# LiXirong/pytorch-r2d2

Measured on AMD Instinct MI355X. Metric: learner_steps_per_sec, higher is better.
Workload: dtype fp32; 1 GPU; model=r2d2-qnet (reference model.py: conv32x3 + LSTM256 + dueling, 6 actions), preset=atari57, global_batch=64, per_gpu_batch=64, seq_len=80, burn_in=40, n_step=5, target_mode=fixed, matmul=bf16x3 split (fp32 accumulate, fp32 state/storage), replay_rows_per_gpu=999936, parallelism=dp1, hip_graph=True, hoisted_step=True, graph_chunk=8

## Files before the change

### csrc/kernels/optim.hip

```cpp
#include "../common.h"
#include "../pack_step.h"
#include "../rms_pack.h"
#include "../adam_elem.h"

__global__ void rmsprop_centered_kernel(float* __restrict__ p, const float* __restrict__ g,
                                        float* __restrict__ sq, float* __restrict__ ga, int64_t n,
                                        float lr, float alpha, float eps, float gscale,
                                        const float* __restrict__ clip_sumsq, float max_norm) {
  float scale = gscale;
  if (clip_sumsq != nullptr && max_norm > 0.f) {
    const float norm = sqrtf(*clip_sumsq) * gscale;
    if (norm > max_norm) scale *= max_norm / (norm + 1e-6f);
  }
  const int64_t n4 = n >> 2;
  const int64_t stride = (int64_t)gridDim.x * blockDim.x;
  for (int64_t i = blockIdx.x * (int64_t)blockDim.x + threadIdx.x; i < n4; i += stride) {
    f32x4 pv = ((f32x4*)p)[i], gv = ((const f32x4*)g)[i];
    f32x4 sv = ((f32x4*)sq)[i], av = ((f32x4*)ga)[i];
#pragma unroll
    for (int e = 0; e < 4; ++e) {
      float s = sv[e], m = av[e];
      pv[e] = rms_elem(s, m, pv[e], gv[e] * scale, lr, alpha, eps);
      sv[e] = s;
      av[e] = m;
    }
    ((f32x4*)p)[i] = pv;
    ((f32x4*)sq)[i] = sv;
    ((f32x4*)ga)[i] = av;
  }
  for (int64_t i = (n4 << 2) + blockIdx.x * (int64_t)blockDim.x + threadIdx.x; i < n; i += stride) {
    float sv = sq[i], av = ga[i];
    p[i] = rms_elem(sv, av, p[i], g[i] * scale, lr, alpha, eps);
    sq[i] = sv;
    ga[i] = av;
  }
}

__global__ __launch_bounds__(256) void rmsprop_pack_kernel(const RmsPackArgs a) {
  const int b = (int)blockIdx.x - a.tblocks;
  if (b < 0) {
    rmsprop_torso_items(a, blockIdx.x);
    return;
  }
  rmsprop_pack_items(a, b * (int64_t)blockDim.x + threadIdx.x, (int64_t)(gridDim.x - a.tblocks) * blockDim.x);
}

__global__ void adam_kernel(float* __restrict__ p, const float* __restrict__ g,
                            float* __restrict__ m, float* __restrict__ v, int64_t n, float lr,
                            float b1, float b2, float eps, float gscale,
                            const int64_t* __restrict__ step, const float* __restrict__ clip_sumsq,
                            float max_norm) {
  float scale = gscale;
  if (clip_sumsq != nullptr && max_norm > 0.f) {
    const float norm = sqrtf(*clip_sumsq) * gscale;
    if (norm > max_norm) scale *= max_norm / (norm + 1e-6f);
  }
  const AdamCoef c = adam_coef(lr, b1, b2, eps, step, 1);
  const int64_t stride = (int64_t)gridDim.x * blockDim.x;
  for (int64_t i = blockIdx.x * (int64_t)blockDim.x + threadIdx.x; i < n; i += stride) {
    float mi = m[i], vi = v[i];
    const float pn = adam_elem(mi, vi, p[i], g[i] * scale, c);
    m[i] = mi;
    v[i] = vi;
    p[i] = pn;
  }
}

__global__ __launch_bounds__(256) void adam_pack_kernel(const RmsPackArgs a, float b2, int step_off) {
  const AdamUpd u{adam_coef(a.lr, a.alpha, b2, a.eps, a.step, step_off)};
  const int b = (int)blockIdx.x - a.tblocks;
  if (b < 0) {
    opt_torso_items(a, blockIdx.x, u);
    return;
  }
  opt_pack_items(a, b * (int64_t)blockDim.x + threadIdx.x, (int64_t)(gridDim.x - a.tblocks) * blockDim.x, u);
}

__global__ void sumsq_kernel(const float* __restrict__ g, int64_t n, float* __restrict__ out) {
  float s = 0.f;
  const int64_t stride = (int64_t)gridDim.x * blockDim.x;
  for (int64_t i = blockIdx.x * (int64_t)blockDim.x + threadIdx.x; i < n; i += stride) s += g[i] * g[i];
  s = wave_sum(s);
  if ((threadIdx.x & 63) == 0) atomicAdd(out, s);
}

constexpr int GSQ_MAX_FLAT = 256;
static inline int gsq_flat_blocks(int64_t quads) {
  int64_t b = (quads + 255) / 256;
  return (int)(b > GSQ_MAX_FLAT ? GSQ_MAX_FLAT : b);
}

__device__ __forceinline__ float gsq_block_sum(float s, float* red) {
  s = wave_sum(s);
  __syncthreads();
  if ((threadIdx.x & 63) == 0) red[threadIdx.x >> 6] = s;
  __syncthreads();
  return ((red[0] + red[1]) + red[2]) + red[3];
}

__global__ __launch_bounds__(256) void grad_sumsq_kernel(
    const float* __restrict__ g, int64_t quads, float* __restrict__ out, float* partials,
    unsigned* ticket, const float* __restrict__ slab, int G, int SL, const int* __restrict__ dst,
    const float* __restrict__ scale, float* __restrict__ gw, int tblocks) {
  __shared__ float part[4][64];
  __shared__ float red[4];
  __shared__ int last;
  float s = 0.f;
  const int b = (int)blockIdx.x - tblocks;
// ... 159 lines not shown
extern "C" int r2_adam_pack(float* p, const float* g, float* m, float* v, int64_t n, float lr,
                            float b1, float b2, float eps, float gscale, const float* clip_sumsq,
                            float max_norm, const int* dst4, bf16* bf, bf16* bf_t, int64_t lo_off,
                            float* target, const int64_t* step, int64_t interval, int step_off,
                            void* stream) {
  RmsPackArgs a{p, g, m, v, n, lr, b1, eps, gscale, clip_sumsq, max_norm, dst4, bf, bf_t,
                lo_off, target, step, interval};
  if (!rms_pack_args_ok(a)) return -1;
  hipLaunchKernelGGL(adam_pack_kernel, dim3(grid_for(n, 4)), dim3(256), 0, (hipStream_t)stream, a,
                     b2, step_off);
  R2_CHECK_LAUNCH();
  return 0;
}

extern "C" int r2_adam_pack_slab(float* p, float* g, float* m, float* v, int64_t n, float lr,
                                 float b1, float b2, float eps, float gscale, const int* dst4,
                                 bf16* bf, bf16* bf_t, int64_t lo_off, float* target,
                                 const int64_t* step, int64_t interval, int step_off,
                                 const float* slab, int grid, int SL, const int* dst,
                                 const float* scale, int64_t tq, void* stream) {
  RmsPackArgs a{p, g, m, v, n, lr, b1, eps, gscale, nullptr, 0.f, dst4, bf, bf_t,
                lo_off, target, step, interval};
  a.slab = slab; a.tdst = dst; a.tscale = scale; a.gw = g;
  a.tG = grid; a.tSL = SL; a.tblocks = (SL + 63) / 64; a.tq = tq;
  if (!rms_pack_args_ok(a) || !slab || !dst || !scale || grid <= 0 || SL <= 0 || tq < 0 ||
      4 * tq > n)
    return -1;
  hipLaunchKernelGGL(adam_pack_kernel, dim3(a.tblocks + grid_for(4 * tq, 4)), dim3(256), 0,
                     (hipStream_t)stream, a, b2, step_off);
  R2_CHECK_LAUNCH();
  return 0;
}

extern "C" int r2_pack_bf16(const float* src, const int* idx, bf16* out, int64_t n, void* stream) {
  hipLaunchKernelGGL(pack_bf16_kernel, dim3(grid_for(n, 2)), dim3(256), 0, (hipStream_t)stream, src,
                     idx, out, n);
  R2_CHECK_LAUNCH();
  return 0;
}

extern "C" int r2_pack_split(const float* src, const int* idx, bf16* out, int64_t n,
                             int64_t lo_off, void* stream) {
  hipLaunchKernelGGL(pack_split_kernel, dim3(grid_for(n, 2)), dim3(256), 0, (hipStream_t)stream,
                     src, idx, out, n, lo_off);
  R2_CHECK_LAUNCH();
  return 0;
}

extern "C" int r2_gather_f32(const float* src, const int* idx, float* out, int64_t n, void* stream) {
  hipLaunchKernelGGL(gather_f32_kernel, dim3(grid_for(n, 2)), dim3(256), 0, (hipStream_t)stream,
                     src, idx, out, n);
  R2_CHECK_LAUNCH();
  return 0;
}

extern "C" int r2_copy_if_due(float* dst, const float* src, int64_t n, const int64_t* step,
                              int64_t interval, void* stream) {
  hipLaunchKernelGGL(copy_if_due_kernel, dim3(grid_for(n, 4)), dim3(256), 0, (hipStream_t)stream,
                     dst, src, n, step, interval);
  R2_CHECK_LAUNCH();
  return 0;
}

__global__ void pack_step_kernel(const PackStepArgs a) {
  pack_step_items(a, blockIdx.x * (int64_t)blockDim.x + threadIdx.x, (int64_t)gridDim.x * blockDim.x);
}
// ... 16 lines not shown
```

### csrc/rms_pack.h

```cpp
#pragma once
#include "common.h"
#include "slab_reduce.h"

struct RmsPackArgs {
  float* p;
  const float* g;
  float* sq;
  float* ga;
  int64_t n;
  float lr, alpha, eps, gscale;
  const float* clip_sumsq;
  float max_norm;
  const int* dst4;
  bf16* bf;
  bf16* bf_t;
  int64_t lo_off;
  float* target;
  const int64_t* step;
  int64_t interval;
  const float* slab;
  const int* tdst;
  const float* tscale;
  float* gw;
  int tG, tSL, tblocks, pad_;
  int64_t tq;
};

__device__ __forceinline__ float rms_elem(float& sq, float& ga, float p, float gr, float lr,
                                          float alpha, float eps) {
  sq = alpha * sq + (1.f - alpha) * gr * gr;
  ga = alpha * ga + (1.f - alpha) * gr;
  return p - lr * gr / (sqrtf(sq - ga * ga) + eps);
}

struct RmsUpd {
  float lr, alpha, eps;
  __device__ __forceinline__ float operator()(float& sq, float& ga, float p, float gr) const {
    return rms_elem(sq, ga, p, gr, lr, alpha, eps);
  }
};

template <class Upd>
__device__ __forceinline__ void opt_pack_items(const RmsPackArgs& a, int64_t first, int64_t stride,
                                               const Upd upd) {
  float scale = a.gscale;
  if (a.clip_sumsq != nullptr && a.max_norm > 0.f) {
    const float norm = sqrtf(*a.clip_sumsq) * a.gscale;
    if (norm > a.max_norm) scale *= a.max_norm / (norm + 1e-6f);
  }
  float* __restrict__ p = a.p;
  const float* __restrict__ g = a.g;
  float* __restrict__ sq = a.sq;
  float* __restrict__ ga = a.ga;
  const bool due = a.interval <= 1 || ((*a.step) + 1) % a.interval == 0;
  const int64_t n = a.n, n4 = n >> 2;
  auto quad = [&](int64_t q) {
    f32x4 pv = ((f32x4*)p)[q], gv = ((const f32x4*)g)[q];
    f32x4 sv = ((f32x4*)sq)[q], av = ((f32x4*)ga)[q];
    const int d = a.dst4[q];
#pragma unroll
    for (int e = 0; e < 4; ++e) {
      float s = sv[e], m = av[e];
      pv[e] = upd(s, m, pv[e], gv[e] * scale);
      sv[e] = s;
      av[e] = m;
    }
    ((f32x4*)p)[q] = pv;
    ((f32x4*)sq)[q] = sv;
    ((f32x4*)ga)[q] = av;
    if (due) ((f32x4*)a.target)[q] = pv;
    if (d >= 0) {
      bf16x4 h, l;
#pragma unroll
      for (int e = 0; e < 4; ++e) {
        h[e] = (bf16)pv[e];
        l[e] = (bf16)(pv[e] - (float)h[e]);
      }
      *(bf16x4*)(a.bf + d) = h;
      if (a.lo_off) *(bf16x4*)(a.bf + a.lo_off + d) = l;
      if (due) {
        *(bf16x4*)(a.bf_t + d) = h;
        if (a.lo_off) *(bf16x4*)(a.bf_t + a.lo_off + d) = l;
      }
    }
  };
  const int64_t qend = a.tblocks ? a.tq : n4;
  for (int64_t i = first; i < qend; i += stride) quad(i);
  for (int64_t i = (n4 << 2) + first; i < n && !a.tblocks; i += stride) {
    float sv = sq[i], av = ga[i];
    p[i] = upd(sv, av, p[i], g[i] * scale);
    sq[i] = sv;
    ga[i] = av;
    if (due) a.target[i] = p[i];
  }
}

__device__ __forceinline__ void rmsprop_pack_items(const RmsPackArgs& a, int64_t first, int64_t stride) {
  opt_pack_items(a, first, stride, RmsUpd{a.lr, a.alpha, a.eps});
}

template <class Upd>
__device__ __forceinline__ void opt_torso_items(const RmsPackArgs& a, int blk, const Upd upd) {
  __shared__ float part[4][64];
  const float s = slab_column_sum(a.slab, a.tG, a.tSL, blk, part);
  const int e = blk * 64 + (int)threadIdx.x;
  if (threadIdx.x >= 64 || e >= a.tSL) return;
  const int m = a.tdst[e];
  const float gv = s * a.tscale[e];
  a.gw[m] = gv;
  float sv = a.sq[m], av = a.ga[m];
  const float pv = upd(sv, av, a.p[m], gv * a.gscale);
  a.sq[m] = sv;
  a.ga[m] = av;
  a.p[m] = pv;
  if (a.interval <= 1 || ((*a.step) + 1) % a.interval == 0) a.target[m] = pv;
}

__device__ __forceinline__ void rmsprop_torso_items(const RmsPackArgs& a, int blk) {
  opt_torso_items(a, blk, RmsUpd{a.lr, a.alpha, a.eps});
}

inline bool rms_pack_args_ok(const RmsPackArgs& a) {
  return !((((uintptr_t)a.p | (uintptr_t)a.g | (uintptr_t)a.sq | (uintptr_t)a.ga | (uintptr_t)a.target) & 15) ||
           (((uintptr_t)a.bf | (uintptr_t)a.bf_t) & 7) || (a.lo_off & 3) || !a.dst4 || !a.step);
}
```

### pytorch_r2d2_amd/config.py

```python
from __future__ import annotations

import copy
import dataclasses
from dataclasses import dataclass, field
from typing import Any, Dict, Optional


@dataclass
class EnvConfig:
    name: str = "synthetic"
    action_repeat: int = 4
    n_stacks: int = 4
    frame_h: int = 84
    frame_w: int = 84
    channels_per_frame: int = 1
    n_actions: int = 6
    episode_len: int = 400
    switch: int = 8
    cue_only_first: bool = False
    obs_dim: int = 4
    pong_points: int = 21
    pong_max_steps: int = 5000
    pong_opp_lapse: int = 64
    breakout_lives: int = 5
# ... 43 lines not shown
    adam_betas: tuple = (0.9, 0.999)
    grad_clip: float = 0.0
    value_rescale: bool = False
    value_rescale_eps: float = 1e-3
    target_update_interval: int = 1000
    publish_interval: int = 100
    ingest_interval: int = 20
    checkpoint_interval: int = 10_000
    initial_exploration: int = 50_000
    target_mode: str = "shifted"
    compute_dtype: str = "bf16"
    lstm_impl: str = "persistent"
    lstm_handoff: str = "tagged"
    bwd_gemm: str = "group"
    fuse_opt_pack: bool = True
    fold_torso_reduce: bool = True
    td_fuse_head_bwd: bool = True
    td_fuse_head_fwd: bool = True
    td_fuse_dh: bool = True
    lstm_xcd_pairs: bool = True
    sp_gemm: str = "fused"
    sp_group_splits: str = "auto"
    sp_group_cfg: int = -2
    sp_head_grads_in_bptt: bool = True
    torso_bwd: str = "fused"
    conv_autotune: bool = True
    use_graph: bool = True
    bptt_dh: bool = True
    hoist: bool = True
    hoist_stop_lead: int = 5
    graph_chunk: int = 8
    hoist_early_fork: bool = True
    fuse_pack_tail: bool = True
    save_dir: str = "save"
    zero_stored_state: bool = False


@dataclass
class ActorConfig:
    n_actors: int = 1
    envs_per_actor: int = 1
    eps_base: float = 0.4
    eps_alpha: float = 7.0
    net_load_interval: int = 5
    memory_save_interval: int = 5
    local_capacity: int = 50_000
    use_graph: bool = True
    return_ring: int = 4096
    reset_state_every_step: bool = False
    clear_ahead: int = 0
    compute_dtype: str = "bf16"


@dataclass
class DistConfig:
    backend: str = "auto"
    grad_bucket_mb: float = 8.0
    grad_dtype: str = "fp32"
    overlap_allreduce: bool = True
    comm_reserve_cus: int = 32
    global_sampling: bool = True
    actor_ranks: int = 0
    push_rows: int = 32
    push_slots: int = 4
    publish_steps: int = 100
    poll_steps: int = 8
# ... 145 lines not shown
```

### pytorch_r2d2_amd/engine/layout.py

```python
from __future__ import annotations

from collections import OrderedDict
from dataclasses import dataclass
from typing import Dict, List, Tuple

import numpy as np
import torch

from ..config import EnvConfig, ModelConfig
from ..models.qnet import torso_dims

UNITS = 16


def gate_perm(H: int) -> np.ndarray:
    nwg = H // UNITS
    j, g, u = np.meshgrid(np.arange(nwg), np.arange(4), np.arange(UNITS), indexing="ij")
    return (g * H + UNITS * j + u).reshape(-1).astype(np.int64)


@dataclass
class Seg:
    name: str
    shape: Tuple[int, ...]
# ... 157 lines not shown

        if self.model.torso == "atari":
            c1, c2, c3 = self.model.conv_channels
            add_f("b1", off("vis_layers.0.bias") + np.arange(c1), (c1,))
            add_f("b2", off("vis_layers.2.bias") + np.arange(c2), (c2,))
            add_f("b3", off("vis_layers.4.bias") + np.arange(c3), (c3,))
        else:
            add_f("mlp_b", off("vis_layers.0.bias") + np.arange(self.D), (self.D,))
        add_f("b_ih", off("lstm.bias_ih") + perm, (G,))
        add_f("b_hh", off("lstm.bias_hh") + perm, (G,))
        add_f("head_b1", off("val.0.bias") + np.arange(2 * HD), (2 * HD,))
        add_f("head_w2", off("val.2.weight") + np.arange((1 + A) * HD), (1 + A, HD))
        add_f("head_b2", off("val.2.bias") + np.arange(1 + A), (1 + A,))
        self.f_numel = cur
        self.f_index = torch.from_numpy(np.concatenate(f).astype(np.int32))
        inv = np.empty_like(perm)
        inv[perm] = np.arange(perm.size)
        self.gate_perm = torch.from_numpy(perm)
        self.gate_inv = torch.from_numpy(inv)

    def _row_dst4(self, idx: np.ndarray, begin: int):
        dst = np.full(self.padded // 4, -1, dtype=np.int64)
        tail = idx[begin:].reshape(-1, 4)
        pad_v = self.segs["lstm.bias_ih"].offset
        run = (tail[:, 0] % 4 == 0) & np.all(np.diff(tail, axis=1) == 1, axis=1)
        q = tail[run, 0] // 4
        if np.unique(q).size != q.size:
            return None
        dst[q] = begin + 4 * np.nonzero(run)[0]
        if not np.all(run | np.all(tail == pad_v, axis=1)):
            return None
        return torch.from_numpy(dst.astype(np.int32))

    def torso_grad_map(self):
        c1, c2, c3 = self.model.conv_channels
        off = lambda n: self.segs[n].offset
        cin = self.cin
        dst, scale = [], []
        dst.append(off("vis_layers.0.weight") + np.arange(c1 * cin * 64))
        scale.append(np.full(c1 * cin * 64, 1.0 / 255.0))
        co, kh, kw, ci = np.meshgrid(np.arange(c2), np.arange(4), np.arange(4), np.arange(c1), indexing="ij")
        dst.append((off("vis_layers.2.weight") + ((co * c1 + ci) * 4 + kh) * 4 + kw).reshape(-1))
        scale.append(np.ones(c2 * 16 * c1))
        co, kh, kw, ci = np.meshgrid(np.arange(c3), np.arange(3), np.arange(3), np.arange(c2), indexing="ij")
        dst.append((off("vis_layers.4.weight") + ((co * c2 + ci) * 3 + kh) * 3 + kw).reshape(-1))
        scale.append(np.ones(c3 * 9 * c2))
        for name, c in (("vis_layers.0.bias", c1), ("vis_layers.2.bias", c2), ("vis_layers.4.bias", c3)):
            dst.append(off(name) + np.arange(c))
            scale.append(np.ones(c))
        return (torch.from_numpy(np.concatenate(dst).astype(np.int32)),
                torch.from_numpy(np.concatenate(scale).astype(np.float32)))

    def packed_views(self, bf: torch.Tensor, f32: torch.Tensor):
        out = {}
        for n, (o, shp) in self.bf_offsets.items():
            out[n] = bf[o:o + int(np.prod(shp))].view(shp)
        for n, (o, shp) in self.f_offsets.items():
            out[n] = f32[o:o + int(np.prod(shp))].view(shp)
        return out

    def pack_torch(self, master: torch.Tensor, bf: torch.Tensor, f32: torch.Tensor) -> None:
        idx = self.bf_index.to(master.device).long()
        bf.copy_(master[idx].to(bf.dtype))
        fidx = self.f_index.to(master.device).long()
        f32.copy_(master[fidx])
```

### pytorch_r2d2_amd/engine/learner_engine.py

```python
from __future__ import annotations

import ctypes
from typing import Dict, List, Optional

import numpy as np
import torch

from ..config import R2D2Config
from ..models.qnet import QNet
from ..ops._lib import bptt_opts, check, kernels, ptr, stream_handle
from ..ops.gemm import G5_CFGS, Gemm, gemm, gemm_group, gemm_sp, gemm_sp_ws_bytes, group_ws_bytes
from ..models.qnet import torso_dims
from ..ops.torso_lib import (fused_torso_fwd_geom, fused_torso_supported, gather_frames_nhwc,
                             torso_backward_library_sp, torso_forward_library,
                             torso_forward_library_sp, torso_fwd_fused)
from .layout import ParamLayout, UNITS
from .replay_hbm import HBMReplay
from .step_driver import StepDrivers, _dispatch_serialized, _graph_upload, dp_hoist_plan


def device_cus(device) -> int:
    d = torch.device(device)
    if d.type != "cuda":
        return 256
# ... 85 lines not shown
            if lstm_wgs > self.n_cus - int(cfg.dist.comm_reserve_cus):
                raise ValueError(
                    f"DP global sampling: the persistent LSTM forward needs {lstm_wgs} co-resident "
                    f"workgroups, more than {self.n_cus} CUs minus dist.comm_reserve_cus="
                    f"{cfg.dist.comm_reserve_cus} left beside the shard-stats all-gather")
        self._duel_done = False
        self._dh_done = False
        self.graph = None
        self.stats: Dict[str, float] = {}
        self._hoist_ready = False
        self._hoist_gen = self._hoist_unc = self._hoist_t = None
        self._hoist_due = False
        self._dev_step_off = None
        self._side = self._gather_stream = None
        self._early_fork = self._early_post = None
        self._early_refused = False
        self._hgraphs, self._hsegs, self._one_graphs = {}, {}, {}
        self._cgraph = self._one_graph = None
        self._one_dp_graph = False
        self.graphs, self._seg_replays = [], []
        self.chunks_run = 0
        self._rollout = self._gsync = None
        self._pack_deferred = None
        self._torso_deferred = False
        self._hprev_sp = self.gg_ws = None
        self._alloc()
        self._fold_tq = None
        if (self.sp and not self.sp_lib and not self.dp and self.world == 1 and lc.fold_torso_reduce
                and self.row_dst4 is not None
                and self.fwd_geom is not None and L.torso_offset % 4 == 0
                and bool((L.row_dst4[L.torso_offset // 4:] < 0).all())):
            self._fold_tq = L.torso_offset // 4
        self._fold_in_norm = bool(self._fold_tq is not None and lc.grad_clip > 0)
        self._pack(always=True)
        if d.type == "cuda":
            torch.cuda.synchronize(d)

    def _alloc(self):
        cfg, d, L = self.cfg, self.device, self.layout
        rc, lc = cfg.replay, cfg.learner
        self.B = B = lc.batch_size
        self.Lb, self.Ll, self.n = rc.burn_in, rc.learn, rc.n_step
        self.T = T = rc.seq_len
        mode = lc.target_mode
        self.mode = mode
        H, D, G, A, HD = L.H, L.D, L.G, L.A, L.HD
        Lb, Ll, n = self.Lb, self.Ll, self.n
        self.Tn = Tn = T + n
        self.Tc = Tn if mode == "shifted" else T
        bf16, f32 = torch.bfloat16, torch.float32
        z = lambda *s, dt=f32: torch.zeros(s, dtype=dt, device=d)
        sp = self.sp

        def zsp(*s):
            if sp:
                t = z(2, *s, dt=bf16)
                return t[0], t[1]
            return z(*s, dt=bf16), None
        act_dt = f32 if sp else bf16
        self.starts = z(B, dt=torch.int32)
        self.probs = z(B)
        self.rows = z(Tn * B, dt=torch.int32)
        self.tq = z(4, dt=torch.int32)
        self.X_on, self.X_on_lo = zsp(Tn * B, D)
        t_lo = 0 if mode == "shifted" else n
        self.t_lo_tg = t_lo
# ... 99 lines not shown
            self.z_nx = z(Nnx, 2 * HD, dt=act_dt)
        self.dh = z(Ll * B, H)
        self.dX, self.dX_lo = zsp(Ll * B, D)
        self.gate_perm_i32 = L.gate_perm.to(d, torch.int32)
        self.gs_ws = torch.zeros(int(kernels().r2_gradsum_ws_floats()), dtype=torch.float32, device=d)
        self.gs_ticket = torch.zeros(64, dtype=torch.int32, device=d)
        if lc.grad_clip > 0:
            self.gsq_part = z(int(kernels().r2_grad_sumsq_partials()))
            self.gsq_ticket = z(1, dt=torch.int32)
        self.dp_recv = z(max(1, self.world) * 3)
        self.dp_params = z(4)

    def _pack(self, always: bool = False, stream=None):
        k = kernels()
        s = stream_handle(stream)
        L = self.layout
        if self.sp:
            check(k.r2_pack_split(ptr(self.master), ptr(self.bf_index), ptr(self.bf), L.bf_numel,
                                  L.bf_numel, s), "pack_split")
        else:
            check(k.r2_pack_bf16(ptr(self.master), ptr(self.bf_index), ptr(self.bf), L.bf_numel, s), "pack")
        check(k.r2_gather_f32(ptr(self.master), ptr(self.f_index), ptr(self.f32), L.f_numel, s), "gather")
        torch.add(self.pk["b_ih"], self.pk["b_hh"], out=self.lstm_b)
        if always:
            if self.sp:
                check(k.r2_pack_split(ptr(self.target), ptr(self.bf_index), ptr(self.bf_t), L.bf_numel,
                                      L.bf_numel, s), "pack_split_t")
            else:
                check(k.r2_pack_bf16(ptr(self.target), ptr(self.bf_index), ptr(self.bf_t), L.bf_numel, s),
                      "pack_t")
            check(k.r2_gather_f32(ptr(self.target), ptr(self.f_index), ptr(self.f32_t), L.f_numel, s), "gather_t")
            torch.add(self.pk_t["b_ih"], self.pk_t["b_hh"], out=self.lstm_b_t)

    def _pack_args(self, interval: int, rows_done: bool):
        L = self.layout
        n_master, n_bf = (0, L.bf_rows_begin) if rows_done else (L.padded, L.bf_numel)
        return (ptr(self.master), ptr(self.target), n_master, ptr(self.bf_index), ptr(self.bf),
                ptr(self.bf_t), n_bf, ptr(self.f_index), ptr(self.f32), ptr(self.f32_t), L.f_numel,
                L.f_offsets["b_ih"][0], L.f_offsets["b_hh"][0], ptr(self.lstm_b), ptr(self.lstm_b_t),
                L.G), (interval, L.bf_numel if self.sp else 0)

    def _pack_step(self, interval: int, s, rows_done: bool = False):
        if self._fuse_pack_tail() and rows_done:
            self._pack_deferred = (interval, rows_done)
            return
        head, tail = self._pack_args(interval, rows_done)
        check(kernels().r2_pack_step(*head, ptr(self.replay.step), *tail, s), "pack_step")

    def _fuse_pack_tail(self) -> bool:
        return (self.cfg.learner.fuse_pack_tail and not self.dp and self.device.type == "cuda"
                and self.cfg.replay.fused_prio_tail and not self.hoist)

    def _hoist_side(self, torso: bool, after_td, td_wait: bool = False):
        side = self._side_stream()
        side.wait_event(after_td)
        rp, B = self.replay, self.B
        nxt = 1 - self._cur
        with torch.cuda.stream(side):
            S, states = self._sample_dst(nxt)
            ok = rp.prio_tail_sample(self.starts, B, self.Lb, self.T, S["starts"], S["probs"],
                                     S["rows"], self.Tn, states, self.sp, self.tq,
                                     skip_xcds=self._bptt_xcds(),
                                     td_wait=self.td_done if td_wait else None,
                                     **({"dp_out": S["dp_send"]} if self.dp_global else {}))
            if not ok and td_wait:
                side.wait_event(self._early_post)
# ... 649 lines not shown
        else:
            gather_frames_nhwc(self.replay.frames, rows, cin, fh, fw, out=self.frames_bf)
        fr = self.frames_bf.view(N, fh, fw, cin).permute(0, 3, 1, 2)
        _, dw1, db1 = cb(g1, fr, w1, [c1], [4, 4], [0, 0], [1, 1], False, [0, 0], 1,
                         [False, True, True])
        if not self.fused_torso:
            dw1 = dw1.float() * (1.0 / 255)
        L.view(g, "vis_layers.4.weight").copy_(dw3)
        L.view(g, "vis_layers.4.bias").copy_(db3)
        L.view(g, "vis_layers.2.weight").copy_(dw2)
        L.view(g, "vis_layers.2.bias").copy_(db2)
        L.view(g, "vis_layers.0.weight").copy_(dw1)
        L.view(g, "vis_layers.0.bias").copy_(db1)

    def _update(self):
        assert self._pack_deferred is None, \
            "a deferred weight repack was never run (_update without _priorities after it)"
        k = kernels()
        s = stream_handle()
        lc, L = self.cfg.learner, self.layout
        n = L.padded
        gscale = 1.0 / self.world
        clip = 0
        slabs = self._fold_tq is not None and self._torso_deferred
        lo_off = L.bf_numel if self.sp else 0
        if lc.grad_clip > 0:
            fold = ((ptr(self._tb_slab), self._tb_grid, int(k.r2_torso_bwd_slab_floats()),
                     ptr(self._tb_dst), ptr(self._tb_scale), ptr(self.grad), self._fold_tq)
                    if slabs else (0, 0, 0, 0, 0, 0, 0))
            check(k.r2_grad_sumsq(ptr(self.grad), n, ptr(self.clip_buf), ptr(self.gsq_part),
                                  ptr(self.gsq_ticket), *fold, s), "grad_sumsq")
            clip = ptr(self.clip_buf)
            slabs = False
        if lc.optimizer == "adam" and self.row_dst4 is None:
            check(k.r2_adam(ptr(self.master), ptr(self.grad), ptr(self.opt_a), ptr(self.opt_b), n,
                            float(lc.lr), float(lc.adam_betas[0]), float(lc.adam_betas[1]),
                            float(lc.eps), gscale, ptr(self.replay.step), clip,
                            float(lc.grad_clip), s), "adam")
        elif lc.optimizer == "adam":
            head = (ptr(self.master), ptr(self.grad), ptr(self.opt_a), ptr(self.opt_b), n,
                    float(lc.lr), float(lc.adam_betas[0]), float(lc.adam_betas[1]), float(lc.eps),
                    gscale)
            tail = (ptr(self.row_dst4), ptr(self.bf), ptr(self.bf_t), lo_off, ptr(self.target),
                    ptr(self.replay.step), self._baked_interval(), self._step_off())
            if slabs:
                check(k.r2_adam_pack_slab(*head, *tail, ptr(self._tb_slab), self._tb_grid,
                                          int(k.r2_torso_bwd_slab_floats()), ptr(self._tb_dst),
                                          ptr(self._tb_scale), self._fold_tq, s), "adam_pack_slab")
            else:
                check(k.r2_adam_pack(*head, clip, float(lc.grad_clip), *tail, s), "adam_pack")
            self._pack_step(self._baked_interval(), s, rows_done=True)
            return
        elif slabs:
            check(k.r2_rmsprop_pack_slab(ptr(self.master), ptr(self.grad), ptr(self.opt_a),
                                         ptr(self.opt_b), n, float(lc.lr), float(lc.rms_alpha),
                                         float(lc.eps), gscale, ptr(self.row_dst4), ptr(self.bf),
                                         ptr(self.bf_t), L.bf_numel if self.sp else 0,
                                         ptr(self.target), ptr(self.replay.step),
                                         self._baked_interval(), ptr(self._tb_slab), self._tb_grid,
                                         int(kernels().r2_torso_bwd_slab_floats()), ptr(self._tb_dst),
                                         ptr(self._tb_scale), self._fold_tq, s), "rmsprop_pack_slab")
            self._pack_step(self._baked_interval(), s, rows_done=True)
            return
        elif self.row_dst4 is not None:
            check(k.r2_rmsprop_pack(ptr(self.master), ptr(self.grad), ptr(self.opt_a),
                                    ptr(self.opt_b), n, float(lc.lr), float(lc.rms_alpha),
# ... 79 lines not shown
```

### pytorch_r2d2_amd/ops/_lib.py

```python
from __future__ import annotations

import ctypes
import os
import threading
from pathlib import Path

import torch

_PKG = Path(__file__).resolve().parent.parent
_SO = _PKG / "_r2d2_kernels.so"
_lock = threading.Lock()
_lib = None

P = ctypes.c_void_p
I = ctypes.c_int
I64 = ctypes.c_int64
U64 = ctypes.c_uint64
F = ctypes.c_float

_SIGS = {
    "r2_abi_version": [],
    "r2_set_num_cus": [I],
    "r2_set_xcd_cus": [P],
    "r2_dp_local_stats": [P, P, P, I, P, P],
# ... 24 lines not shown
    "r2_lstm_bwd_tag_sp_hg": [P, P, P, P, P, P, P, P, I, I, I, I, P, P, P, P, P, P, P,
                              P, P, P, P, P, P, P, I, I, I, P, P, P, P],
    "r2_tree_sample": [P, P, P, I, I, U64, P, P, P, P],
    "r2_tree_rebuild": [P, P, P, I, P],
    "r2_tree_update": [P, P, P, I, P, P, I, P],
    "r2_tree_update_fused": [P, P, P, I, P, P, I, P, P, P],
    "r2_tree_update_fused_reset": [P, P, P, I, P, P, I, P, P],
    "r2_seqprio_refresh": [P, I, P, P, P, I, I, I, I, F, P, P, I, P],
    "r2_mark_starts": [P, P, I, P, P, P, I, I, F, P, P, P, I, P],
    "r2_hoist_guard": [P, I, P, P, P, I, I, I, I, P, I, P, P],
    "r2_make_rows": [P, I, I, I, I, P, P],
    "r2_sample_batch": [P, P, P, I, I, U64, P, P, P, P, I, I, I, I, P, P, P, P, P],
    "r2_sample_batch_f32h": [P, P, P, I, I, U64, P, P, P, P, I, I, I, I, P, P, P, P, P],
    "r2_sample_batch_q": [P, P, P, I, I, U64, P, P, P, P, I, I, I, I, P, P, P, P, I, P, P],
    "r2_torso_fwd_sp_multi": [P, P, I, I, P],
    "r2_torso_sp_debug": [I],
    "r2_torso_sp_trace": [P],
    "r2_torso_bwd_sp_trace": [P],
    "r2_torso_bwd_sp_debug": [I],
    "r2_torso_bwd_sp": [P, P, I, P, P, P, P, P, P, P, P, P, P, P, P, I, P, P, P, P],
    "r2_torso_grad_reduce": [P, I, P, P, P, P],
    "r2_gather_state": [P, P, I, I, I, I, P, P, P, P],
    "r2_step_end": [P, P, P],
    "r2_rmsprop_centered": [P, P, P, P, I64, F, F, F, F, P, F, P],
    "r2_rmsprop_pack": [P, P, P, P, I64, F, F, F, F, P, F, P, P, P, I64, P, P, I64, P],
    "r2_rmsprop_pack_slab": [P, P, P, P, I64, F, F, F, F, P, P, P, I64, P, P, I64, P, I, I, P, P, I64, P],
    "r2_adam": [P, P, P, P, I64, F, F, F, F, F, P, P, F, P],
    "r2_sumsq": [P, I64, P, P],
    "r2_grad_sumsq": [P, I64, P, P, P, P, I, I, P, P, P, I64, P],
    "r2_grad_sumsq_partials": [],
    "r2_adam_pack": [P, P, P, P, I64, F, F, F, F, F, P, F, P, P, P, I64, P, P, I64, I, P],
    "r2_adam_pack_slab": [P, P, P, P, I64, F, F, F, F, F, P, P, P, I64, P, P, I64, I, P, I, I, P, P,
                          I64, P],
    "r2_pack_bf16": [P, P, P, I64, P],
    "r2_gather_f32": [P, P, P, I64, P],
    "r2_copy_if_due": [P, P, I64, P, I64, P],
    "r2_noop_chain": [P, I, I, P],
    "r2_torso_bwd": [P, P, I, P, P, P, P, P, P, P, I, P, P, P, P],
    "r2_torso_bwd_slab_floats": [],
    "r2_torso_bwd_geom": [P, I64, P, I, P, P, P, P, P, P, P, I, P, P, P, I, I, I, P],
    "r2_torso_bwd_slab_floats_geom": [I, I, I],
    "r2_gemm": [P, I, P],
    "r2_gemm_set_version": [I],
    "r2_gemm_group": [P, P, I, P, I64, P, I, P],
    "r2_gemm_group_ws_bytes": [P, P, I],
    "r2_dueling_fwd_multi": [P, I, I, I, P],
    "r2_actor_pre": [P, P],
    "r2_actor_post": [P, P],
    "r2_actor_tail": [P, P],
    "r2_actor_args_bytes": [],
    "r2_eval_act": [P, P],
    "r2_eval_post": [P, P],
    "r2_eval_args_bytes": [],
    "r2_pack_step": [P, P, I64, P, P, P, I64, P, P, P, I64, I64, I64, P, P, I64, P, I64, I64, P],
    "r2_pack_split": [P, P, P, I64, I64, P],
    "r2_torso_bwd_set_debug": [P],
    "r2_torso_fwd_set_debug": [P],
    "r2_lstm_persist_set_debug": [P],
    "r2_lstm_fwd_set_stamps": [P],
    "r2_prio_tail": [P, I, P, P, P, P, P, I, I, I, I, I, F, P, P, I, P, P, I, P],
    "r2_lstm_bptt_opts_bytes": [],
    "r2_lstm_probes": [],
    "r2_prio_tail_sample": [P, I, P, P, P, P, P, I, I, I, I, I, F, P, P, I, P, P, U64, P, P, P, I,
                            I, I, P, P, P, P, I, P, I, P, P],
    "r2_prio_tail_sample_dp": [P, I, P, P, P, P, P, I, I, I, I, I, F, P, P, I, P, P, U64, P, P, P, I,
                               I, I, P, P, P, P, I, P, I, P, P, P, P],
# ... 128 lines not shown
```

Before: 1144 learner steps/s of the whole job, one step = a 64 x 80-step sequence batch (= optimizer steps/s x 1 ranks; global batch 64).

## Fold tail packing of torso, LSTM bias and head params into optimizer kernel

Adds fold tables so the fused optimizer+pack kernel also writes bf16 split copies and fp32 copies for torso weights, LSTM biases (summed b_ih+b_hh) and head params. A transposed scatter path handles LSTM w_hh and head weights, and a new block range handles small items. This replaces the separate pack-tail step (the gather_f32 and bias-add launches) with extra scattered writes inside one kernel. It adds uncoalesced byte writes and a deal() index permutation in exchange for fewer launches and less re-reading of master params.

```diff
diff --git a/csrc/kernels/optim.hip b/csrc/kernels/optim.hip
--- a/csrc/kernels/optim.hip
+++ b/csrc/kernels/optim.hip
@@ -37,12 +37,7 @@
 }
 
 __global__ __launch_bounds__(256) void rmsprop_pack_kernel(const RmsPackArgs a) {
-  const int b = (int)blockIdx.x - a.tblocks;
-  if (b < 0) {
-    rmsprop_torso_items(a, blockIdx.x);
-    return;
-  }
-  rmsprop_pack_items(a, b * (int64_t)blockDim.x + threadIdx.x, (int64_t)(gridDim.x - a.tblocks) * blockDim.x);
+  opt_pack_blocks(a, RmsUpd{a.lr, a.alpha, a.eps});
 }
 
 __global__ void adam_kernel(float* __restrict__ p, const float* __restrict__ g,
@@ -67,13 +62,7 @@
 }
 
 __global__ __launch_bounds__(256) void adam_pack_kernel(const RmsPackArgs a, float b2, int step_off) {
-  const AdamUpd u{adam_coef(a.lr, a.alpha, b2, a.eps, a.step, step_off)};
-  const int b = (int)blockIdx.x - a.tblocks;
-  if (b < 0) {
-    opt_torso_items(a, blockIdx.x, u);
-    return;
-  }
-  opt_pack_items(a, b * (int64_t)blockDim.x + threadIdx.x, (int64_t)(gridDim.x - a.tblocks) * blockDim.x, u);
+  opt_pack_blocks(a, AdamUpd{adam_coef(a.lr, a.alpha, b2, a.eps, a.step, step_off)});
 }
 
 __global__ void sumsq_kernel(const float* __restrict__ g, int64_t n, float* __restrict__ out) {
@@ -299,6 +288,67 @@
   return 0;
 }
 
+static int opt_fold_fill(RmsPackArgs& a, float* g, const float* slab, int grid, int SL, const int* dst,
+                         const float* scale, int64_t tq, const int64_t* fold) {
+  if (!rms_pack_args_ok(a) || !dst || SL <= 0 || tq < 0 || 4 * tq > a.n || !fold) return -1;
+  if (slab && (!scale || grid <= 0)) return -1;
+  a.slab = slab; a.tdst = dst; a.tscale = scale; a.gw = g;
+  a.tG = grid; a.tSL = SL; a.tblocks = (SL + 63) / 64; a.tq = tq;
+  a.tpk = (const int*)fold[0];
+  a.f32 = (float*)fold[1]; a.f32_t = (float*)fold[2];
+  a.lstm_b = (float*)fold[3]; a.lstm_b_t = (float*)fold[4];
+  a.sm = (const int*)fold[5];
+  a.n_sm = (int)fold[6];
+  a.sblocks = (a.n_sm + 255) / 256;
+  if (!a.tpk || !a.f32 || !a.f32_t || !a.lstm_b || !a.lstm_b_t || !a.sm || a.n_sm <= 0 ||
+      fold[6] > (1 << 24) || ((uintptr_t)a.sm & 15))
+    return -1;
+  a.dstT = (const int*)fold[7];
+  a.tT_q0 = fold[8]; a.tT_q1 = fold[9]; a.tT_split = fold[10];
+  a.tT_s0 = (int)fold[11]; a.tT_s1 = (int)fold[12];
+  a.tT_mid = fold[13];
+  a.tT_qr = (int)fold[14];
+  if (!a.dstT || a.tT_q0 < 0 || a.tT_q1 < a.tT_q0 || a.tT_q1 > tq || a.tT_s0 <= 0 || a.tT_s1 <= 0)
+    return -1;
+  if (a.tT_qr <= 0 || (a.tT_qr & 3) || fold[14] > (1 << 20) || a.tT_mid < a.tT_q0 ||
+      a.tT_split < a.tT_mid || a.tT_split > a.tT_q1 || (a.tT_mid - a.tT_q0) % (16 * a.tT_qr) ||
+      (a.tT_q1 - a.tT_split) % (16 * a.tT_qr))
+    return -1;
+  return 0;
+}
+
+extern "C" int r2_rmsprop_pack_fold(float* p, float* g, float* sq, float* ga, int64_t n, float lr,
+                                    float alpha, float eps, float gscale, const float* clip_sumsq,
+                                    float max_norm, const int* dst4, bf16* bf, bf16* bf_t,
+                                    int64_t lo_off, float* target, const int64_t* step,
+                                    int64_t interval, const float* slab, int grid, int SL,
+                                    const int* dst, const float* scale, int64_t tq,
+                                    const int64_t* fold, void* stream) {
+  RmsPackArgs a{p, g, sq, ga, n, lr, alpha, eps, gscale, clip_sumsq, max_norm, dst4, bf, bf_t,
+                lo_off, target, step, interval};
+  if (opt_fold_fill(a, g, slab, grid, SL, dst, scale, tq, fold)) return -1;
+  hipLaunchKernelGGL(rmsprop_pack_kernel, dim3(a.tblocks + a.sblocks + grid_for(4 * tq, 4)),
+                     dim3(256), 0, (hipStream_t)stream, a);
+  R2_CHECK_LAUNCH();
+  return 0;
+}
+
+extern "C" int r2_adam_pack_fold(float* p, float* g, float* m, float* v, int64_t n, float lr,
+                                 float b1, float b2, float eps, float gscale,
+                                 const float* clip_sumsq, float max_norm, const int* dst4, bf16* bf,
+                                 bf16* bf_t, int64_t lo_off, float* target, const int64_t* step,
+                                 int64_t interval, int step_off, const float* slab, int grid, int SL,
+                                 const int* dst, const float* scale, int64_t tq,
+                                 const int64_t* fold, void* stream) {
+  RmsPackArgs a{p, g, m, v, n, lr, b1, eps, gscale, clip_sumsq, max_norm, dst4, bf, bf_t,
+                lo_off, target, step, interval};
+  if (opt_fold_fill(a, g, slab, grid, SL, dst, scale, tq, fold)) return -1;
+  hipLaunchKernelGGL(adam_pack_kernel, dim3(a.tblocks + a.sblocks + grid_for(4 * tq, 4)),
+                     dim3(256), 0, (hipStream_t)stream, a, b2, step_off);
+  R2_CHECK_LAUNCH();
+  return 0;
+}
+
 extern "C" int r2_pack_bf16(const float* src, const int* idx, bf16* out, int64_t n, void* stream) {
   hipLaunchKernelGGL(pack_bf16_kernel, dim3(grid_for(n, 2)), dim3(256), 0, (hipStream_t)stream, src,
                      idx, out, n);
diff --git a/csrc/rms_pack.h b/csrc/rms_pack.h
--- a/csrc/rms_pack.h
+++ b/csrc/rms_pack.h
@@ -24,7 +24,32 @@
   float* gw;
   int tG, tSL, tblocks, pad_;
   int64_t tq;
+  const int* tpk;
+  float* f32;
+  float* f32_t;
+  float* lstm_b;
+  float* lstm_b_t;
+  const int* sm;
+  int n_sm, sblocks;
+  const int* dstT;
+  int64_t tT_q0, tT_q1, tT_split;
+  int tT_s0, tT_s1;
+  int64_t tT_mid;
+  int tT_qr, pad2_;
 };
+
+__device__ __forceinline__ float opt_scale(const RmsPackArgs& a) {
+  float scale = a.gscale;
+  if (a.clip_sumsq != nullptr && a.max_norm > 0.f) {
+    const float norm = sqrtf(*a.clip_sumsq) * a.gscale;
+    if (norm > a.max_norm) scale *= a.max_norm / (norm + 1e-6f);
+  }
+  return scale;
+}
+
+__device__ __forceinline__ bool opt_due(const RmsPackArgs& a) {
+  return a.interval <= 1 || ((*a.step) + 1) % a.interval == 0;
+}
 
 __device__ __forceinline__ float rms_elem(float& sq, float& ga, float p, float gr, float lr,
                                           float alpha, float eps) {
@@ -43,21 +68,18 @@
 template <class Upd>
 __device__ __forceinline__ void opt_pack_items(const RmsPackArgs& a, int64_t first, int64_t stride,
                                                const Upd upd) {
-  float scale = a.gscale;
-  if (a.clip_sumsq != nullptr && a.max_norm > 0.f) {
-    const float norm = sqrtf(*a.clip_sumsq) * a.gscale;
-    if (norm > a.max_norm) scale *= a.max_norm / (norm + 1e-6f);
-  }
+  const float scale = opt_scale(a);
   float* __restrict__ p = a.p;
   const float* __restrict__ g = a.g;
   float* __restrict__ sq = a.sq;
   float* __restrict__ ga = a.ga;
-  const bool due = a.interval <= 1 || ((*a.step) + 1) % a.interval == 0;
+  const bool due = opt_due(a);
   const int64_t n = a.n, n4 = n >> 2;
   auto quad = [&](int64_t q) {
     f32x4 pv = ((f32x4*)p)[q], gv = ((const f32x4*)g)[q];
     f32x4 sv = ((f32x4*)sq)[q], av = ((f32x4*)ga)[q];
     const int d = a.dst4[q];
+    if (d == -2) return;
 #pragma unroll
     for (int e = 0; e < 4; ++e) {
       float s = sv[e], m = av[e];
@@ -82,10 +104,34 @@
         *(bf16x4*)(a.bf_t + d) = h;
         if (a.lo_off) *(bf16x4*)(a.bf_t + a.lo_off + d) = l;
       }
-    }
+      if (a.dstT && q >= a.tT_q0 && q < a.tT_q1) {
+        const int t = a.dstT[q - a.tT_q0];
+        const int st = q < a.tT_split ? a.tT_s0 : a.tT_s1;
+        if (t >= 0) {
+#pragma unroll
+          for (int e = 0; e < 4; ++e) {
+            a.bf[t + e * st] = h[e];
+            if (a.lo_off) a.bf[a.lo_off + t + e * st] = l[e];
+            if (due) {
+              a.bf_t[t + e * st] = h[e];
+              if (a.lo_off) a.bf_t[a.lo_off + t + e * st] = l[e];
+            }
+          }
+        }
+      }
+    }
+  };
+  auto deal = [&](int64_t i) {
+    if (!a.dstT || i < a.tT_q0 || i >= a.tT_q1) return i;
+    const int64_t base = i < a.tT_mid ? a.tT_q0 : a.tT_split;
+    if (i >= a.tT_mid && i < a.tT_split) return i;
+    const int64_t r = i - base, tile = r >> 6;
+    const int lane = (int)(r & 63), per = a.tT_qr >> 2;
+    const int64_t row = (tile / per) * 16 + (lane & 15);
+    return base + row * a.tT_qr + (tile % per) * 4 + (lane >> 4);
   };
   const int64_t qend = a.tblocks ? a.tq : n4;
-  for (int64_t i = first; i < qend; i += stride) quad(i);
+  for (int64_t i = first; i < qend; i += stride) quad(deal(i));
   for (int64_t i = (n4 << 2) + first; i < n && !a.tblocks; i += stride) {
     float sv = sq[i], av = ga[i];
     p[i] = upd(sv, av, p[i], g[i] * scale);
@@ -102,22 +148,86 @@
 template <class Upd>
 __device__ __forceinline__ void opt_torso_items(const RmsPackArgs& a, int blk, const Upd upd) {
   __shared__ float part[4][64];
-  const float s = slab_column_sum(a.slab, a.tG, a.tSL, blk, part);
+  const float s = a.slab ? slab_column_sum(a.slab, a.tG, a.tSL, blk, part) : 0.f;
   const int e = blk * 64 + (int)threadIdx.x;
   if (threadIdx.x >= 64 || e >= a.tSL) return;
   const int m = a.tdst[e];
-  const float gv = s * a.tscale[e];
-  a.gw[m] = gv;
+  float gv;
+  if (a.slab) {
+    gv = s * a.tscale[e];
+    a.gw[m] = gv;
+  } else {
+    gv = a.g[m];
+  }
   float sv = a.sq[m], av = a.ga[m];
-  const float pv = upd(sv, av, a.p[m], gv * a.gscale);
+  const float pv = upd(sv, av, a.p[m], gv * opt_scale(a));
   a.sq[m] = sv;
   a.ga[m] = av;
   a.p[m] = pv;
-  if (a.interval <= 1 || ((*a.step) + 1) % a.interval == 0) a.target[m] = pv;
-}
-
-__device__ __forceinline__ void rmsprop_torso_items(const RmsPackArgs& a, int blk) {
-  opt_torso_items(a, blk, RmsUpd{a.lr, a.alpha, a.eps});
+  const bool due = opt_due(a);
+  if (due) a.target[m] = pv;
+  if (!a.tpk) return;
+  const bf16 h = (bf16)pv;
+  const bf16 l = (bf16)(pv - (float)h);
+#pragma unroll
+  for (int k = 0; k < 2; ++k) {
+    const int d = a.tpk[k * a.tSL + e];
+    if (d < 0) continue;
+    a.bf[d] = h;
+    if (a.lo_off) a.bf[d + a.lo_off] = l;
+    if (due) {
+      a.bf_t[d] = h;
+      if (a.lo_off) a.bf_t[d + a.lo_off] = l;
+    }
+  }
+  const int d = a.tpk[2 * a.tSL + e];
+  if (d >= 0) {
+    a.f32[d] = pv;
+    if (due) a.f32_t[d] = pv;
+  }
+}
+
+template <class Upd>
+__device__ __forceinline__ void opt_small_items(const RmsPackArgs& a, int i, const Upd upd) {
+  if (i >= a.n_sm) return;
+  const float scale = opt_scale(a);
+  const bool due = opt_due(a);
+  const int4 it = ((const int4*)a.sm)[i];
+  auto one = [&](int m, int d) {
+    float sv = a.sq[m], av = a.ga[m];
+    const float pv = upd(sv, av, a.p[m], a.g[m] * scale);
+    a.sq[m] = sv;
+    a.ga[m] = av;
+    a.p[m] = pv;
+    if (due) a.target[m] = pv;
+    if (d >= 0) {
+      a.f32[d] = pv;
+      if (due) a.f32_t[d] = pv;
+    }
+    return pv;
+  };
+  const float pa = one(it.x, it.y);
+  if (it.z < 0) return;
+  const float pb = one(it.z, it.w);
+  const float b = pa + pb;
+  a.lstm_b[i] = b;
+  if (due) a.lstm_b_t[i] = b;
+}
+
+template <class Upd>
+__device__ __forceinline__ void opt_pack_blocks(const RmsPackArgs& a, const Upd upd) {
+  int b = (int)blockIdx.x - a.tblocks;
+  if (b < 0) {
+    opt_torso_items(a, blockIdx.x, upd);
+    return;
+  }
+  b -= a.sblocks;
+  if (b < 0) {
+    opt_small_items(a, (b + a.sblocks) * (int)blockDim.x + (int)threadIdx.x, upd);
+    return;
+  }
+  opt_pack_items(a, b * (int64_t)blockDim.x + threadIdx.x,
+                 (int64_t)(gridDim.x - a.tblocks - a.sblocks) * blockDim.x, upd);
 }
 
 inline bool rms_pack_args_ok(const RmsPackArgs& a) {
diff --git a/pytorch_r2d2_amd/config.py b/pytorch_r2d2_amd/config.py
--- a/pytorch_r2d2_amd/config.py
+++ b/pytorch_r2d2_amd/config.py
@@ -99,6 +99,7 @@
     graph_chunk: int = 8
     hoist_early_fork: bool = True
     fuse_pack_tail: bool = True
+    fuse_pack_opt: bool = True
     save_dir: str = "save"
     zero_stored_state: bool = False
 
diff --git a/pytorch_r2d2_amd/engine/layout.py b/pytorch_r2d2_amd/engine/layout.py
--- a/pytorch_r2d2_amd/engine/layout.py
+++ b/pytorch_r2d2_amd/engine/layout.py
@@ -213,6 +213,81 @@
             return None
         return torch.from_numpy(dst.astype(np.int32))
 
+    def fold_tables(self):
+        if self.model.torso != "atari" or self.row_dst4 is None or self.numel != self.padded:
+            return None
+        off = lambda n: self.segs[n].offset
+        dst = self.torso_grad_map()[0].numpy().astype(np.int64)
+        SL, t0 = dst.size, self.torso_offset
+        if SL != self.numel - t0 or np.unique(dst).size != SL or dst.min() < t0:
+            return None
+        e_of = np.full(self.padded, -1, dtype=np.int64)
+        e_of[dst] = np.arange(SL)
+        tpk = np.full((3, SL), -1, dtype=np.int64)
+        conv_end, rows = self.bf_offsets["w_hhT"][0], self.bf_rows_begin
+        bi = self.bf_index.numpy().astype(np.int64)
+        fi = self.f_index.numpy().astype(np.int64)
+        if bool((bi[conv_end:] >= t0).any()) or conv_end % 4 or rows % 4:
+            return None
+        pos = np.nonzero(bi[:conv_end] >= t0)[0]
+        order = np.argsort(e_of[bi[pos]], kind="stable")
+        es, ps = e_of[bi[pos]][order], pos[order]
+        first = np.r_[True, es[1:] != es[:-1]]
+        rank = np.arange(es.size) - np.maximum.accumulate(np.where(first, np.arange(es.size), 0))
+        if rank.max() > 1:
+            return None
+        tpk[rank, es] = ps
+        fpos = np.nonzero(fi >= t0)[0]
+        fe = e_of[fi[fpos]]
+        if np.unique(fe).size != fe.size:
+            return None
+        tpk[2, fe] = fpos
+        G, perm = self.G, gate_perm(self.H)
+        bih, bhh, s0 = off("lstm.bias_ih"), off("lstm.bias_hh"), off("val.0.bias")
+        if bih % 4 or s0 % 4 or bhh != bih + G or G % 4:
+            return None
+        o_bih, o_bhh = self.f_offsets["b_ih"][0], self.f_offsets["b_hh"][0]
+        j = np.arange(G)
+        bias = np.stack([bih + perm, o_bih + j, bhh + perm, o_bhh + j], axis=1)
+        slot = np.full(self.padded, -1, dtype=np.int64)
+        hpos = np.arange(self.f_offsets["head_b1"][0], self.f_numel)
+        hpos = hpos[fi[hpos] >= s0]
+        if np.unique(fi[hpos]).size != hpos.size or hpos.size != self.core_numel - s0:
+            return None
+        slot[fi[hpos]] = hpos
+        m = np.arange(s0, t0)
+        rest = np.stack([m, slot[m], np.full(m.size, -1), np.full(m.size, -1)], axis=1)
+        sm = np.concatenate([bias, rest]).astype(np.int32)
+        dst4 = self.row_dst4.numpy().copy()
+        own = np.r_[np.arange(bih // 4, (bhh + G) // 4), np.arange(s0 // 4, t0 // 4)]
+        if bool((dst4[own] != -1).any()):
+            return None
+        dst4[own] = -2
+        q0, q1, split = off("lstm.weight_hh") // 4, s0 // 4, off("val.0.weight") // 4
+        strides = (UNITS * 4, 2 * self.HD)
+        if off("lstm.weight_hh") % 4 or off("val.0.weight") % 4 or self.H % 16 \
+                or G % 16 or (2 * self.HD) % 16 or bih != off("lstm.weight_hh") + G * self.H:
+            return None
+        tpos = np.arange(conv_end, rows)
+        tpos = tpos[bi[tpos] != bih]
+        at = np.full(self.padded, -1, dtype=np.int64)
+        if np.unique(bi[tpos]).size != tpos.size:
+            return None
+        at[bi[tpos]] = tpos
+        qs = np.arange(q0, q1)
+        base = at[4 * qs]
+        st = np.where(qs < split, strides[0], strides[1])
+        has = base >= 0
+        for e in range(1, 4):
+            if bool((at[4 * qs + e][has] != (base + e * st)[has]).any()) \
+                    or bool((at[4 * qs + e][~has] >= 0).any()):
+                return None
+        if 4 * int(has.sum()) != tpos.size or bool((dst4[qs][has] < 0).any()):
+            return None
+        return dict(tpk=torch.from_numpy(tpk.astype(np.int32)), sm=torch.from_numpy(sm),
+                    dst4=torch.from_numpy(dst4), dstT=torch.from_numpy(base.astype(np.int32)),
+                    tT=(q0, q1, split) + strides + (bih // 4, self.H // 4), SL=SL)
+
     def torso_grad_map(self):
         c1, c2, c3 = self.model.conv_channels
         off = lambda n: self.segs[n].offset
diff --git a/pytorch_r2d2_amd/engine/learner_engine.py b/pytorch_r2d2_amd/engine/learner_engine.py
--- a/pytorch_r2d2_amd/engine/learner_engine.py
+++ b/pytorch_r2d2_amd/engine/learner_engine.py
@@ -141,6 +141,7 @@
                 and bool((L.row_dst4[L.torso_offset // 4:] < 0).all())):
             self._fold_tq = L.torso_offset // 4
         self._fold_in_norm = bool(self._fold_tq is not None and lc.grad_clip > 0)
+        self._fold_pack = self._fold_pack_tables()
         self._pack(always=True)
         if d.type == "cuda":
             torch.cuda.synchronize(d)
@@ -306,6 +307,23 @@
             check(k.r2_gather_f32(ptr(self.target), ptr(self.f_index), ptr(self.f32_t), L.f_numel, s), "gather_t")
             torch.add(self.pk_t["b_ih"], self.pk_t["b_hh"], out=self.lstm_b_t)
 
+    def _fold_pack_tables(self):
+        lc, L, d = self.cfg.learner, self.layout, self.device
+        if not (lc.fuse_pack_opt and self.hoist and not self.dp and self.world == 1
+                and d.type == "cuda" and self.sp and self.fused_torso and not self.sp_lib
+                and self.row_dst4 is not None and self._fold_tq is not None
+                and self._dh_in_bptt()):
+            return None
+        t = L.fold_tables()
+        if t is None or t["SL"] != int(kernels().r2_torso_bwd_slab_floats()) \
+                or t["SL"] != self._tb_dst.numel():
+            return None
+        f = dict(tpk=t["tpk"].to(d), sm=t["sm"].to(d), dst4=t["dst4"].to(d), dstT=t["dstT"].to(d))
+        f["opt"] = np.asarray([ptr(f["tpk"]), ptr(self.f32), ptr(self.f32_t), ptr(self.lstm_b),
+                               ptr(self.lstm_b_t), ptr(f["sm"]), f["sm"].shape[0], ptr(f["dstT"]),
+                               *t["tT"]], dtype=np.int64)
+        return f
+
     def _pack_args(self, interval: int, rows_done: bool):
         L = self.layout
         n_master, n_bf = (0, L.bf_rows_begin) if rows_done else (L.padded, L.bf_numel)
@@ -1021,6 +1039,22 @@
                                   ptr(self.gsq_ticket), *fold, s), "grad_sumsq")
             clip = ptr(self.clip_buf)
             slabs = False
+        if self._fold_pack is not None:
+            f = self._fold_pack
+            slab = ((ptr(self._tb_slab), self._tb_grid) if slabs else (0, 0)) + (
+                self._tb_dst.numel(), ptr(self._tb_dst), ptr(self._tb_scale), self._fold_tq,
+                f["opt"].ctypes.data, s)
+            mid = (ptr(f["dst4"]), ptr(self.bf), ptr(self.bf_t), lo_off, ptr(self.target),
+                   ptr(self.replay.step), self._baked_interval())
+            head = (ptr(self.master), ptr(self.grad), ptr(self.opt_a), ptr(self.opt_b), n, float(lc.lr))
+            if lc.optimizer == "adam":
+                check(k.r2_adam_pack_fold(*head, float(lc.adam_betas[0]), float(lc.adam_betas[1]),
+                                          float(lc.eps), gscale, clip, float(lc.grad_clip), *mid,
+                                          self._step_off(), *slab), "adam_pack_fold")
+            else:
+                check(k.r2_rmsprop_pack_fold(*head, float(lc.rms_alpha), float(lc.eps), gscale, clip,
+                                             float(lc.grad_clip), *mid, *slab), "rmsprop_pack_fold")
+            return
         if lc.optimizer == "adam" and self.row_dst4 is None:
             check(k.r2_adam(ptr(self.master), ptr(self.grad), ptr(self.opt_a), ptr(self.opt_b), n,
                             float(lc.lr), float(lc.adam_betas[0]), float(lc.adam_betas[1]),
diff --git a/pytorch_r2d2_amd/ops/_lib.py b/pytorch_r2d2_amd/ops/_lib.py
--- a/pytorch_r2d2_amd/ops/_lib.py
+++ b/pytorch_r2d2_amd/ops/_lib.py
@@ -80,6 +80,10 @@
     "r2_adam_pack": [P, P, P, P, I64, F, F, F, F, F, P, F, P, P, P, I64, P, P, I64, I, P],
     "r2_adam_pack_slab": [P, P, P, P, I64, F, F, F, F, F, P, P, P, I64, P, P, I64, I, P, I, I, P, P,
                           I64, P],
+    "r2_rmsprop_pack_fold": [P, P, P, P, I64, F, F, F, F, P, F, P, P, P, I64, P, P, I64, P, I, I, P, P,
+                             I64, P, P],
+    "r2_adam_pack_fold": [P, P, P, P, I64, F, F, F, F, F, P, F, P, P, P, I64, P, P, I64, I, P, I, I, P,
+                          P, I64, P, P],
     "r2_pack_bf16": [P, P, P, I64, P],
     "r2_gather_f32": [P, P, P, I64, P],
     "r2_copy_if_due": [P, P, I64, P, I64, P],
```

Result: no change. 1146 learner steps/s of the whole job, one step = a 64 x 80-step sequence batch (= optimizer steps/s x 1 ranks; global batch 64), median of 3 (+0.2%).
